# happierpig/flashinfer-ai

Hardware: AMD Instinct MI355X
Metric: paged_decode_hbm_bandwidth_bs64_kv8192_hd128 (higher is better)
Workload: dtype bf16; 1 GPU; C2: BatchDecodeWithPagedKVCacheWrapper bf16 GQA 32/8 head_dim=128 page_size=16 bs=64/GPU kv_len=8192, random page permutation; batch_per_gpu=64, kv_len=8192, num_qo_heads=32, num_kv_heads=8, head_dim=128, page_size=16, split_kv=True, kv_chunk_size=4096, parallelism=batch-shard x1 (no data-path collective)

## Files before the change

flashinfer-ai_amd/csrc/decode.hip:

```cpp
#include <stdlib.h>
#include <string.h>

#include <algorithm>
#include <vector>

#include "decode_kernel.h"
#include "merge_kernel.h"

namespace fi {

#define FI_DECL(DT, HD)                                                                   \
  hipError_t decode_launch_##DT##_##HD(const DecodeKernelParams& p, int gt, int rope, int grid, \
                                       hipStream_t stream);
FI_DECL(0, 64) FI_DECL(0, 128) FI_DECL(0, 256) FI_DECL(0, 512)
FI_DECL(1, 64) FI_DECL(1, 128) FI_DECL(1, 256) FI_DECL(1, 512)
FI_DECL(2, 64) FI_DECL(2, 128) FI_DECL(2, 256) FI_DECL(2, 512)
FI_DECL(3, 64) FI_DECL(3, 128) FI_DECL(3, 256) FI_DECL(3, 512)
#undef FI_DECL

typedef hipError_t (*decode_launch_fn)(const DecodeKernelParams&, int, int, int, hipStream_t);

static decode_launch_fn find_launcher(int kv_dt, int head_dim) {
#define FI_ROW(DT)                          \
  case DT:                                  \
    switch (head_dim) {                     \
      case 64:                              \
        return decode_launch_##DT##_64;     \
      case 128:                             \
        return decode_launch_##DT##_128;    \
      case 256:                             \
        return decode_launch_##DT##_256;    \
      case 512:                             \
        return decode_launch_##DT##_512;    \
      default:                              \
        return nullptr;                     \
    }
  switch (kv_dt) {
    FI_ROW(0)
    FI_ROW(1)
    FI_ROW(2)
    FI_ROW(3)
    default:
      return nullptr;
  }
#undef FI_ROW
}

static bool decode_mfma16() {
  static const bool on = [] {
    const char* e = getenv("FI_DECODE_MFMA16");
    return !e || atoi(e) != 0;
  }();
  return on;
}

static int decode_waves_per_cu(int kv_dtype, bool batch) {
  const bool fp8 = kv_dtype == FI_DTYPE_FP8_E4M3 || kv_dtype == FI_DTYPE_FP8_E5M2;
  return (batch && !fp8) ? 4 : 8;
}

static int tokens_per_load(int kv_dt, int head_dim) {
  const int vec = 16 / (int)dtype_size(kv_dt);
  return 64 / (head_dim / vec);
}

static int ilog2_exact(int x) {
  if (x <= 0 || (x & (x - 1))) return -1;
  int l = 0;
  while ((1 << l) < x) ++l;
  return l;
}

hipError_t decode_mfma_launch(const DecodeKernelParams& p, int q_dtype, int kv_dtype, int head_dim, int rope, int grid,
                              hipStream_t stream);
hipError_t decode_mfma16_launch(const DecodeKernelParams& p, int q_dtype, int kv_dtype, int head_dim, int rope,
                                int grid, hipStream_t stream);

constexpr int kMfmaMinGroup = 5;
constexpr int kMfmaMinGroupFp8 = 3;

enum class DecodeKernel { VALU, MFMA32, MFMA16 };

struct DecodeChoice {
  DecodeKernel kind;
  int head_tiles;
  int gt;
};

static DecodeChoice choose_decode(int group, int q_dt, int kv_dt, int head_dim, int page_size, bool rope,
                                  bool plain_logits, bool strides_fit_31_bits) {
  DecodeChoice c;
  c.gt = group <= 1 ? 1 : group == 2 ? 2 : 4;
  const bool fp8 = kv_dt == FI_DTYPE_FP8_E4M3 || kv_dt == FI_DTYPE_FP8_E5M2;
  const bool mfma = (q_dt == FI_DTYPE_F16 || q_dt == FI_DTYPE_BF16) && (kv_dt == q_dt || fp8) &&
                    (head_dim == 64 || head_dim == 128) && strides_fit_31_bits;
  if (decode_mfma16()) {
    c.kind = !(mfma && (plain_logits || group <= 16)) ? DecodeKernel::VALU
             : group <= 16                            ? DecodeKernel::MFMA16
                                                      : DecodeKernel::MFMA32;
  } else {
    const bool small_pages = ilog2_exact(page_size) < 0 || page_size < tokens_per_load(kv_dt, head_dim);
    const int min_group = (rope || small_pages) ? 1 : fp8 ? kMfmaMinGroupFp8 : kMfmaMinGroup;
    c.kind = mfma && plain_logits && group >= min_group ? DecodeKernel::MFMA32 : DecodeKernel::VALU;
  }
  c.head_tiles = c.kind == DecodeKernel::VALU ? ceil_div(group, c.gt) : ceil_div(group, 32);
  return c;
}

static int launch_decode(const DecodeKernelParams& kp, const DecodeChoice& c, int q_dt, int kv_dt, int head_dim,
                         bool rope, int merge_n, int merge_rows, hipStream_t stream) {
  if (kp.num_items > 0) {
    const int grid = ceil_div(kp.num_items, kDecodeWaves);
    if (c.kind == DecodeKernel::MFMA16)
      FI_HIP_CALL(decode_mfma16_launch(kp, q_dt, kv_dt, head_dim, rope, grid, stream));
    else if (c.kind == DecodeKernel::MFMA32)
      FI_HIP_CALL(decode_mfma_launch(kp, q_dt, kv_dt, head_dim, rope, grid, stream));
    else
      FI_HIP_CALL(find_launcher(kv_dt, head_dim)(kp, c.gt, rope, grid, stream));
  }
  if (kp.split_kv) {
    MergeNParams mp{kp.tmp_o, kp.tmp_lse, kp.o_indptr, kp.o, kp.lse, merge_n, merge_rows,
                    kp.num_qo_heads, head_dim, FI_DTYPE_F32, q_dt};
    FI_HIP_CALL(launch_merge_n(mp, stream));
  }
  return 0;
}

static int32_t window_pages(const int32_t* indptr_h, int i, int page_size, int window_left) {
  const int32_t np = indptr_h[i + 1] - indptr_h[i];
  if (window_left < 0 || np <= 0) return np;
  const int64_t first = std::max<int64_t>((int64_t)(np - 1) * page_size - window_left, 0) / page_size;
  return (int32_t)(np - first);
}

struct DecodeWork {
  bool split_kv;
  uint32_t pages_per_chunk;
  size_t padded;
};

static DecodeWork estimate_decode_work(const int32_t* indptr_h, int batch_size, int page_size, int window_left,
                                       uint32_t gdy, uint32_t max_grid, bool enable_cuda_graph) {
  std::vector<int32_t> num_pages(batch_size);
  uint32_t max_pages = 0;
  for (int i = 0; i < batch_size; ++i)
    max_pages = std::max<uint32_t>(max_pages, num_pages[i] = window_pages(indptr_h, i, page_size, window_left));
  if ((uint64_t)batch_size * gdy >= max_grid) return {false, std::max(max_pages, 1u), (size_t)batch_size};
  const uint32_t min_pages = std::max<uint32_t>(128u / (uint32_t)page_size, 1u);
  const uint32_t pages_per_chunk = (uint32_t)smallest_fitting(min_pages, max_pages, [&](int64_t pages) {
    uint64_t nb = 0;
    for (int32_t e : num_pages) nb += ceil_div<uint32_t>((uint32_t)e, (uint32_t)pages);
    return nb * gdy > max_grid;
  });
  uint32_t new_batch = 0;
  for (int32_t e : num_pages) new_batch += ceil_div<uint32_t>((uint32_t)std::max(e, 1), pages_per_chunk);
  if (enable_cuda_graph) return {true, pages_per_chunk, std::max<size_t>(max_grid / gdy, new_batch)};
  return {new_batch != (uint32_t)batch_size, pages_per_chunk, new_batch};
}

}

using namespace fi;

extern "C" FI_API int fi_batch_decode_plan(void* float_ws, size_t float_ws_bytes, void* int_ws,
                                    void* pinned_int_ws, size_t int_ws_bytes,
                                    const int32_t* indptr_h, int32_t batch_size,
                                    int32_t num_qo_heads, int32_t num_kv_heads, int32_t page_size,
                                    int32_t enable_cuda_graph, int32_t head_dim, int32_t q_dtype,
                                    int32_t kv_dtype, int32_t max_grid_hint, int32_t window_left,
                                    int64_t* plan_info_out, fi_stream_t stream) {
  (void)float_ws;
  FI_REQUIRE(pinned_int_ws && indptr_h && plan_info_out, "batch_decode_plan: null argument");
  FI_REQUIRE(batch_size >= 0 && page_size > 0, "batch_decode_plan: bad batch_size/page_size");
  FI_REQUIRE(num_kv_heads > 0 && num_qo_heads % num_kv_heads == 0,
             "batch_decode_plan: num_qo_heads (%d) must be a multiple of num_kv_heads (%d)",
             num_qo_heads, num_kv_heads);
  FI_REQUIRE(q_dtype == FI_DTYPE_F16 || q_dtype == FI_DTYPE_BF16,
             "batch_decode_plan: q dtype must be f16/bf16");
  FI_REQUIRE(find_launcher(kv_dtype, head_dim) != nullptr,
             "batch_decode_plan: unsupported kv dtype %d / head_dim %d", kv_dtype, head_dim);
  for (int i = 0; i < batch_size; ++i)
    FI_REQUIRE(indptr_h[i + 1] >= indptr_h[i], "batch_decode_plan: indptr must be non-decreasing");

  const int head_tiles = choose_decode(num_qo_heads / num_kv_heads, q_dtype, kv_dtype, head_dim, page_size,
                                       false, true, true)
                             .head_tiles;
  const uint32_t gdy = (uint32_t)(num_kv_heads * head_tiles);
  const uint32_t max_grid =
      max_grid_hint > 0 ? (uint32_t)max_grid_hint
                        : (uint32_t)(fi_num_compute_units() * decode_waves_per_cu(kv_dtype, true) * (head_tiles > 1 ? 2 : 1));

  if (window_left < 0) window_left = -1;
  const auto [split_kv, pages_per_chunk, padded] =
      estimate_decode_work(indptr_h, batch_size, page_size, window_left, gdy, max_grid, enable_cuda_graph);

  OffsetAllocator ia(int_ws_bytes);
  const int64_t req_off = ia.alloc(padded * sizeof(int32_t));
  const int64_t tile_off = ia.alloc(padded * sizeof(int32_t));
  const int64_t oind_off = ia.alloc(((size_t)batch_size + 1) * sizeof(int32_t));
  const int64_t chunk_off = ia.alloc(sizeof(int32_t));
  int64_t mask_off = 0;
  if (split_kv) mask_off = ia.alloc(padded);
  FI_REQUIRE(ia.ok, "batch_decode_plan: int workspace too small (%zu bytes)", int_ws_bytes);

  char* hp = (char*)pinned_int_ws;
  int32_t* req_h = (int32_t*)(hp + req_off);
  int32_t* tile_h = (int32_t*)(hp + tile_off);
  int32_t* oind_h = (int32_t*)(hp + oind_off);
  memset(req_h, 0, padded * sizeof(int32_t));
  memset(tile_h, 0, padded * sizeof(int32_t));
  size_t w = 0;
  oind_h[0] = 0;
  for (int b = 0; b < batch_size; ++b) {
    const uint32_t np = (uint32_t)std::max(window_pages(indptr_h, b, page_size, window_left), 1);
    const uint32_t nchunks = split_kv ? ceil_div(np, pages_per_chunk) : 1u;
    for (uint32_t t = 0; t < nchunks; ++t) {
      FI_REQUIRE(w < padded, "batch_decode_plan: work list overflow");
      req_h[w] = b;
      tile_h[w] = (int32_t)t;
      ++w;
    }
    oind_h[b + 1] = oind_h[b] + (int32_t)nchunks;
  }
  *(int32_t*)(hp + chunk_off) = (int32_t)(pages_per_chunk * (uint32_t)page_size);
  if (split_kv) {
    uint8_t* mask_h = (uint8_t*)(hp + mask_off);
    for (size_t i = 0; i < padded; ++i) mask_h[i] = i < w;
  }

  int64_t v_off = 0, s_off = 0;
  if (split_kv) {
    OffsetAllocator fa(float_ws_bytes);
    v_off = fa.alloc((size_t)num_qo_heads * padded * head_dim * sizeof(float));
    s_off = fa.alloc((size_t)num_qo_heads * padded * sizeof(float));
    FI_REQUIRE(fa.ok, "batch_decode_plan: float workspace too small (%zu bytes, need %zu)",
               float_ws_bytes, (size_t)num_qo_heads * padded * (head_dim + 1) * sizeof(float));
  }

  for (int i = 0; i < FI_DECODE_PLAN_INFO_LEN; ++i) plan_info_out[i] = 0;
  plan_info_out[FI_DP_PADDED_BATCH_SIZE] = (int64_t)padded;
  plan_info_out[FI_DP_V_OFFSET] = v_off;
  plan_info_out[FI_DP_S_OFFSET] = s_off;
  plan_info_out[FI_DP_REQUEST_INDICES_OFFSET] = req_off;
  plan_info_out[FI_DP_KV_TILE_INDICES_OFFSET] = tile_off;
  plan_info_out[FI_DP_O_INDPTR_OFFSET] = oind_off;
  plan_info_out[FI_DP_BLOCK_VALID_MASK_OFFSET] = mask_off;
  plan_info_out[FI_DP_KV_CHUNK_SIZE_PTR_OFFSET] = chunk_off;
  plan_info_out[FI_DP_ENABLE_CUDA_GRAPH] = enable_cuda_graph ? 1 : 0;
  plan_info_out[FI_DP_SPLIT_KV] = split_kv ? 1 : 0;
  plan_info_out[FI_DP_KV_CHUNK_SIZE] = (int64_t)pages_per_chunk * page_size;
  plan_info_out[FI_DP_NUM_WORK] = (int64_t)w;
  plan_info_out[FI_DP_BATCH_SIZE] = batch_size;
  plan_info_out[FI_DP_INT_BYTES_USED] = (int64_t)ia.used;
  plan_info_out[FI_DP_WINDOW_LEFT] = window_left;
  plan_info_out[FI_DP_MAGIC] = FI_DECODE_PLAN_MAGIC;

  if (int_ws && ia.used)
    FI_HIP_CALL(hipMemcpyAsync(int_ws, pinned_int_ws, ia.used, hipMemcpyHostToDevice,
                               (hipStream_t)stream));
  return 0;
}

namespace fi {

template <class A>
static int check_and_fill_decode(const char* who, const A& a, int kv_dt, int head_dim, int num_kv_heads,
                                 int page_size, int64_t kv_stride_page, int64_t kv_stride_n, int64_t kv_stride_h,
                                 DecodeKernelParams& kp, DecodeChoice& choice) {
  FI_REQUIRE(a.q_dtype == FI_DTYPE_F16 || a.q_dtype == FI_DTYPE_BF16, "%s: q dtype must be f16/bf16", who);
  FI_REQUIRE(num_kv_heads > 0 && a.num_qo_heads % num_kv_heads == 0,
             "%s: num_qo_heads must be a multiple of num_kv_heads", who);
  FI_REQUIRE(find_launcher(kv_dt, head_dim), "%s: unsupported kv dtype %d / head_dim %d", who, kv_dt, head_dim);
  FI_REQUIRE(a.pos_encoding_mode != FI_POS_ALIBI || a.alibi_slopes, "%s: ALIBI needs alibi_slopes", who);
  memset(&kp, 0, sizeof(kp));
  kp.q = a.q;
  kp.o = a.o;
  kp.lse = a.lse;
  kp.alibi_slopes = a.alibi_slopes;
  kp.kv_stride_page = kv_stride_page;
  kp.kv_stride_n = kv_stride_n;
  kp.kv_stride_h = kv_stride_h;
  kp.num_qo_heads = a.num_qo_heads;
  kp.num_kv_heads = num_kv_heads;
  kp.group_size = a.num_qo_heads / num_kv_heads;
  kp.page_size = page_size;
  kp.log2_page_size = ilog2_exact(page_size);
  kp.uniform_page = kp.log2_page_size >= 0 && page_size >= tokens_per_load(kv_dt, head_dim);
  kp.page_div = FastDiv((uint32_t)page_size);
  kp.window_left = a.window_left;
  kp.q_dtype = a.q_dtype;
  kp.use_alibi = a.pos_encoding_mode == FI_POS_ALIBI;
  kp.logits_soft_cap = a.logits_soft_cap > 0.f ? a.logits_soft_cap : 0.f;
  kp.sm_scale = a.sm_scale;
  kp.rope_rcp_scale = a.rope_rcp_scale;
  kp.rope_rcp_theta = a.rope_rcp_theta;
  const bool plain_logits = a.pos_encoding_mode != FI_POS_ALIBI && !(a.logits_soft_cap > 0.f);
  choice = choose_decode(kp.group_size, a.q_dtype, kv_dt, head_dim, page_size,
                         a.pos_encoding_mode == FI_POS_ROPE_LLAMA, plain_logits,
                         kv_stride_page < (1ll << 31) && kv_stride_n < (1ll << 31));
  kp.head_tiles = choice.head_tiles;
  return 0;
}

}

extern "C" FI_API int fi_batch_decode_run(void* float_ws, size_t float_ws_bytes, void* int_ws,
                                   size_t int_ws_bytes, const int64_t* plan_info,
                                   int32_t plan_info_len, const fi_batch_decode_params_t* a,
                                   fi_stream_t stream_) {
  hipStream_t stream = (hipStream_t)stream_;
  FI_REQUIRE(plan_info && plan_info_len == FI_DECODE_PLAN_INFO_LEN &&
                 plan_info[FI_DP_MAGIC] == FI_DECODE_PLAN_MAGIC,
             "batch_decode_run: plan_info is not a decode plan (call plan() first)");
  FI_REQUIRE(a && a->q && a->o && a->kv.k_data && a->kv.v_data && a->kv.indptr &&
                 a->kv.last_page_len,
             "batch_decode_run: null tensor");
  FI_REQUIRE(int_ws, "batch_decode_run: null int workspace");
  const fi_paged_kv_t& kv = a->kv;
  FI_REQUIRE(kv.batch_size == plan_info[FI_DP_BATCH_SIZE],
             "batch_decode_run: batch size %d differs from the planned %lld", kv.batch_size,
             (long long)plan_info[FI_DP_BATCH_SIZE]);
  FI_REQUIRE(a->pos_encoding_mode >= 0 && a->pos_encoding_mode <= 2,
             "batch_decode_run: bad pos_encoding_mode %d", a->pos_encoding_mode);
  DecodeKernelParams kp;
  DecodeChoice choice;
  if (check_and_fill_decode("batch_decode_run", *a, kv.dtype, kv.head_dim, kv.num_kv_heads, kv.page_size,
                            kv.stride_page, kv.stride_n, kv.stride_h, kp, choice))
    return 1;
  const size_t esz = dtype_size(kv.dtype);
  FI_REQUIRE(((uintptr_t)a->q % 16) == 0 && (a->q_stride_n * 2) % 16 == 0 && (a->q_stride_h * 2) % 16 == 0,
             "batch_decode_run: q rows must be 16-byte aligned");
  FI_REQUIRE((kv.stride_n * esz) % 16 == 0 && (kv.stride_h * esz) % 16 == 0 &&
                 (kv.stride_page * esz) % 16 == 0 && ((uintptr_t)kv.k_data % 16) == 0 &&
                 ((uintptr_t)kv.v_data % 16) == 0,
             "batch_decode_run: kv cache rows must be 16-byte aligned");
  if (kv.batch_size == 0) return 0;

  const bool split = plan_info[FI_DP_SPLIT_KV] != 0;
  const int64_t padded = plan_info[FI_DP_PADDED_BATCH_SIZE];
  kp.k = kv.k_data;
  kp.v = kv.v_data;
  kp.indptr = kv.indptr;
  kp.indices = kv.indices;
  kp.last_page_len = kv.last_page_len;
  const char* ib = (const char*)int_ws;
  kp.request_indices = (const int32_t*)(ib + plan_info[FI_DP_REQUEST_INDICES_OFFSET]);
  kp.kv_tile_indices = (const int32_t*)(ib + plan_info[FI_DP_KV_TILE_INDICES_OFFSET]);
  kp.o_indptr = (const int32_t*)(ib + plan_info[FI_DP_O_INDPTR_OFFSET]);
  kp.block_valid_mask =
      (split && plan_info[FI_DP_ENABLE_CUDA_GRAPH])
          ? (const uint8_t*)(ib + plan_info[FI_DP_BLOCK_VALID_MASK_OFFSET])
          : nullptr;
  (void)int_ws_bytes;
  kp.q_rope_offset = a->q_rope_offset;
  kp.kv_rope_pos_offset = kv.rope_pos_offset;
  kp.q_stride_n = a->q_stride_n;
  kp.q_stride_h = a->q_stride_h;
  kp.num_items = (int32_t)(padded * kv.num_kv_heads * kp.head_tiles);
  kp.kv_chunk_size = (int32_t)plan_info[FI_DP_KV_CHUNK_SIZE];
  kp.kv_chunk_size_ptr = (const int32_t*)(ib + plan_info[FI_DP_KV_CHUNK_SIZE_PTR_OFFSET]);
  kp.split_kv = split;
  kp.plan_window_left = (int32_t)plan_info[FI_DP_WINDOW_LEFT];
  FI_REQUIRE(kp.plan_window_left < 0 || kp.plan_window_left == a->window_left,
             "batch_decode_run: window_left %d differs from the planned %d", a->window_left, kp.plan_window_left);
  if (split) {
    FI_REQUIRE(float_ws, "batch_decode_run: split-kv plan needs the float workspace");
    const size_t need = (size_t)plan_info[FI_DP_S_OFFSET] +
                        (size_t)a->num_qo_heads * padded * sizeof(float);
    FI_REQUIRE(need <= float_ws_bytes, "batch_decode_run: float workspace too small");
    kp.tmp_o = (float*)((char*)float_ws + plan_info[FI_DP_V_OFFSET]);
    kp.tmp_lse = (float*)((char*)float_ws + plan_info[FI_DP_S_OFFSET]);
  }
  kp.fast_path = kp.uniform_page && kp.indices && !kp.use_alibi && kp.logits_soft_cap == 0.f;
  return launch_decode(kp, choice, a->q_dtype, kv.dtype, kv.head_dim, a->pos_encoding_mode == FI_POS_ROPE_LLAMA,
                       0, kv.batch_size, stream);
}

extern "C" FI_API int fi_single_decode_run(const fi_single_decode_params_t* a, void* tmp, size_t tmp_bytes,
                                    fi_stream_t stream_) {
  hipStream_t stream = (hipStream_t)stream_;
  FI_REQUIRE(a && a->q && a->k && a->v && a->o, "single_decode_run: null tensor");
  FI_REQUIRE(a->kv_len >= 0, "single_decode_run: negative kv_len");
  const int vpage = 16;
  DecodeKernelParams kp;
  DecodeChoice choice;
  if (check_and_fill_decode("single_decode_run", *a, a->kv_dtype, a->head_dim, a->num_kv_heads, vpage,
                            (int64_t)vpage * a->kv_stride_n, a->kv_stride_n, a->kv_stride_h, kp, choice))
    return 1;
  const size_t esz = dtype_size(a->kv_dtype);
  FI_REQUIRE(((uintptr_t)a->q % 16) == 0 && (a->q_stride_h * 2) % 16 == 0,
             "single_decode_run: q rows must be 16-byte aligned");
  FI_REQUIRE((a->kv_stride_n * esz) % 16 == 0 && (a->kv_stride_h * esz) % 16 == 0 &&
                 ((uintptr_t)a->k % 16) == 0 && ((uintptr_t)a->v % 16) == 0,
             "single_decode_run: k/v rows must be 16-byte aligned");

  kp.k = a->k;
  kp.v = a->v;
  kp.q_stride_n = 0;
  kp.q_stride_h = a->q_stride_h;
  kp.single_kv_len = a->kv_len;
  kp.plan_window_left = -1;
  const int gdy = a->num_kv_heads * kp.head_tiles;
  const int max_grid = fi_num_compute_units() * decode_waves_per_cu(a->kv_dtype, false);
  int chunk = a->kv_len, nchunks = 1;
  if (a->kv_len > 256 && tmp) {
    const int want = std::max(1, max_grid / gdy);
    chunk = std::max(ceil_div(a->kv_len, want), 256);
    chunk = ceil_div(chunk, vpage) * vpage;
    nchunks = ceil_div(a->kv_len, chunk);
    const size_t need = (size_t)nchunks * a->num_qo_heads * (a->head_dim + 1) * sizeof(float) + 64;
    if (need > tmp_bytes || nchunks <= 1) {
      chunk = a->kv_len;
      nchunks = 1;
    }
  }
  kp.split_kv = nchunks > 1;
  kp.kv_chunk_size = chunk;
  kp.num_items = nchunks * gdy;
  if (kp.split_kv) {
    kp.tmp_o = (float*)tmp;
    size_t vbytes = (size_t)nchunks * a->num_qo_heads * a->head_dim * sizeof(float);
    vbytes = (vbytes + 15) / 16 * 16;
    kp.tmp_lse = (float*)((char*)tmp + vbytes);
  }
  return launch_decode(kp, choice, a->q_dtype, a->kv_dtype, a->head_dim, a->pos_encoding_mode == FI_POS_ROPE_LLAMA,
                       nchunks, 1, stream);
}
```

flashinfer-ai_amd/csrc/decode_kernel.h:

```cpp
#pragma once
#include "common.h"

namespace fi {

constexpr int kDecodeThreads = 256;
constexpr int kDecodeWaves = kDecodeThreads / 64;
constexpr float kMInit = -1.0e30f;

struct DecodeKernelParams {
  const void* q;
  void* o;
  float* lse;
  float* tmp_o;
  float* tmp_lse;
  const void* k;
  const void* v;
  const int32_t* indptr;
  const int32_t* indices;
  const int32_t* last_page_len;
  const int32_t* request_indices;
  const int32_t* kv_tile_indices;
  const int32_t* o_indptr;
  const uint8_t* block_valid_mask;
  const int32_t* q_rope_offset;
  const int32_t* kv_rope_pos_offset;
  const float* alibi_slopes;
  int64_t q_stride_n, q_stride_h;
  int64_t kv_stride_page, kv_stride_n, kv_stride_h;
  int32_t num_items;
  int32_t num_qo_heads, num_kv_heads, group_size, head_tiles;
  int32_t page_size, log2_page_size;
  int32_t uniform_page;
  int32_t fast_path;
  FastDiv page_div;
  int32_t kv_chunk_size;
  const int32_t* kv_chunk_size_ptr;
  int32_t split_kv;
  int32_t single_kv_len;
  int32_t window_left;
  int32_t plan_window_left;
  int32_t q_dtype;
  int32_t use_alibi;
  float logits_soft_cap;
  float sm_scale;
  float rope_rcp_scale, rope_rcp_theta;
};

template <bool NT>
__device__ __forceinline__ u32x4 load16(const void* base, int64_t byte_off) {
  if constexpr (NT) return __builtin_nontemporal_load((const u32x4*)((const char*)base + byte_off));
  else return *(const u32x4*)((const char*)base + byte_off);
}
template <bool NT>
__device__ __forceinline__ u32x4 load16(const char* ubase, uint32_t lane_byte_off) {
  if constexpr (NT) return __builtin_nontemporal_load((const u32x4*)(ubase + lane_byte_off));
  else return *(const u32x4*)(ubase + lane_byte_off);
}

template <int KV_DT, int HEAD_DIM, int GT, bool ROPE, bool FAST, int NLOAD, bool NT = true>
struct DecodeWave {
  using T = KVTraits<KV_DT>;
  static constexpr int VEC = T::VEC;
  static constexpr int LPT = HEAD_DIM / VEC;
  static constexpr int TPL = 64 / LPT;
  static constexpr int TILE = NLOAD * TPL;
  static_assert(LPT >= 1 && LPT <= 64 && (64 % LPT) == 0, "bad head_dim");

  const DecodeKernelParams& p;
  int lane, c, r;
  int kv_head, page_begin, kv_len, chunk_start, chunk_end, win_start;
  int64_t head_off;
  uint32_t lane_voff;
  int rope_pos0;
  float q[GT][VEC];
  float o[GT][VEC];
  float m[GT], d[GT];
  float slope_l2[GT];
  float s_scale;
  float freq[ROPE ? VEC : 1];
  float rc[ROPE ? VEC : 1], rs[ROPE ? VEC : 1];
  float dc[ROPE ? VEC : 1], ds[ROPE ? VEC : 1];

  __device__ __forceinline__ DecodeWave(const DecodeKernelParams& params) : p(params) {}

  struct Buf {
    u32x4 k[NLOAD];
    u32x4 v[NLOAD];
  };

  template <bool SCALAR>
  __device__ __forceinline__ void fetch_pages(int tile_tok0, int (&pg)[NLOAD]) const {
#pragma unroll
    for (int j = 0; j < NLOAD; ++j) {
      const int tok0 = tile_tok0 + j * TPL;
      if constexpr (SCALAR) {
        const int pi = min(tok0, chunk_end - 1) >> p.log2_page_size;
        pg[j] = p.indices[page_begin + pi];
      } else {
        const int tok = min(tok0 + r, chunk_end - 1);
        const int pi = (int)fast_div((uint32_t)tok, p.page_div);
        pg[j] = p.indices ? p.indices[page_begin + pi] : pi;
      }
    }
  }

  template <bool SCALAR>
  __device__ __forceinline__ void issue_loads(int tile_tok0, const int (&pg)[NLOAD], Buf& b) const {
#pragma unroll
    for (int j = 0; j < NLOAD; ++j) {
      const int tok0 = tile_tok0 + j * TPL;
      if constexpr (SCALAR) {
        const int page = __builtin_amdgcn_readfirstlane(pg[j]);
        const int entry0 = tok0 & (p.page_size - 1);
        const int64_t sbase =
            ((int64_t)page * p.kv_stride_page + head_off + (int64_t)entry0 * p.kv_stride_n) * T::BYTES;
        b.k[j] = load16<NT>((const char*)p.k + sbase, lane_voff);
        b.v[j] = load16<NT>((const char*)p.v + sbase, lane_voff);
      } else {
        const int tok = min(tok0 + r, chunk_end - 1);
        const int pi = (int)fast_div((uint32_t)tok, p.page_div);
        const int entry = tok - pi * p.page_size;
        const int64_t off = (int64_t)pg[j] * p.kv_stride_page + head_off +
                            (int64_t)entry * p.kv_stride_n + (int64_t)(c * VEC);
        b.k[j] = load16<NT>(p.k, off * T::BYTES);
        b.v[j] = load16<NT>(p.v, off * T::BYTES);
      }
    }
  }

  static __device__ __forceinline__ void unpack_q(const u32x4 (&raw)[VEC / 8], bool is_bf16,
                                                  float (&out)[VEC]) {
#pragma unroll
    for (int v8 = 0; v8 < VEC / 8; ++v8) {
      float a[8], b[8];
      KVTraits<FI_DTYPE_BF16>::unpack(raw[v8], a);
      KVTraits<FI_DTYPE_F16>::unpack(raw[v8], b);
#pragma unroll
      for (int i = 0; i < 8; ++i) out[8 * v8 + i] = is_bf16 ? a[i] : b[i];
    }
  }

  __device__ __forceinline__ void rope_seed(int pos) {
    if constexpr (ROPE) {
#pragma unroll
      for (int i = 0; i < VEC; ++i) {
        float e = (float)pos * freq[i];
        float sn, cs;
        sincos_ool(e, &sn, &cs);
        rc[i] = cs;
        rs[i] = sn;
      }
    }
  }
  __device__ __forceinline__ void rope_advance() {
    if constexpr (ROPE) {
#pragma unroll
      for (int i = 0; i < VEC; ++i) {
        float cn = rc[i] * dc[i] - rs[i] * ds[i];
        float sn = rs[i] * dc[i] + rc[i] * ds[i];
        rc[i] = cn;
        rs[i] = sn;
      }
    }
  }

  template <bool MASKED>
  __device__ __forceinline__ void compute(int tile_tok0, const Buf& b) {
    float s[NLOAD][GT];
#pragma unroll
    for (int j = 0; j < NLOAD; ++j) {
      float kf[VEC];
      T::unpack(b.k[j], kf);
      if constexpr (ROPE) {
        float kr[VEC];
#pragma unroll
        for (int i = 0; i < VEC; ++i) {
          float partner = lane_xor<LPT / 2>(kf[i]);
          kr[i] = kf[i] * rc[i] + ((c < LPT / 2) ? -partner : partner) * rs[i];
        }
#pragma unroll
        for (int i = 0; i < VEC; ++i) kf[i] = kr[i];
        rope_advance();
      }
      const int tok = tile_tok0 + j * TPL + r;
#pragma unroll
      for (int g = 0; g < GT; ++g) {
        f32x2 acc2 = {0.f, 0.f};
#pragma unroll
        for (int i = 0; i < VEC; i += 2) {
          f32x2 qq = {q[g][i], q[g][i + 1]};
          f32x2 kk = {kf[i], kf[i + 1]};
          acc2 = __builtin_elementwise_fma(qq, kk, acc2);
        }
        float acc = group_sum<LPT>(acc2[0] + acc2[1]);
        if constexpr (!FAST) {
          if (p.use_alibi) acc += slope_l2[g] * (float)tok;
          if (p.logits_soft_cap > 0.f) acc = fast_tanh(acc) * s_scale;
        }
        if constexpr (MASKED) {
// ... 273 lines not shown
```

flashinfer-ai_amd/csrc/decode_mfma16_kernel.h:

```cpp
#pragma once
#include "decode_kernel.h"
#include "prefill_kernel.h"

namespace fi {

template <int T16>
struct Mfma16;
template <>
struct Mfma16<FI_DTYPE_F16> {
  static __device__ __forceinline__ f32x4 mfma(MfmaType<FI_DTYPE_F16>::frag a, MfmaType<FI_DTYPE_F16>::frag b, f32x4 c) {
    return __builtin_amdgcn_mfma_f32_16x16x32_f16(a, b, c, 0, 0, 0);
  }
};
template <>
struct Mfma16<FI_DTYPE_BF16> {
  static __device__ __forceinline__ f32x4 mfma(MfmaType<FI_DTYPE_BF16>::frag a, MfmaType<FI_DTYPE_BF16>::frag b, f32x4 c) {
    return __builtin_amdgcn_mfma_f32_16x16x32_bf16(a, b, c, 0, 0, 0);
  }
};

template <bool MAX>
__device__ __forceinline__ float reduce_rows(float x) {
  const uint32_t u = __builtin_bit_cast(uint32_t, x);
  const auto r = __builtin_amdgcn_permlane16_swap(u, u, false, false);
// ... 205 lines not shown
#pragma unroll
      for (int e = 0; e < 4; ++e) {
        const float cn = rc[e4 + e] * dc4[e] - rs[e4 + e] * ds4[e];
        const float sn = rs[e4 + e] * dc4[e] + rc[e4 + e] * ds4[e];
        rc[e4 + e] = cn;
        rs[e4 + e] = sn;
      }
    }
  };
  auto write_stage = [&](const Stage& st) {
#pragma unroll
    for (int ps = 0; ps < NPASS; ++ps) {
      const int row = ps * RPP + st_row;
      if constexpr (KV_FP8) {
        u32x4 k0 = fp8x8_to_16<T16, KVS>(u32x2{st.k[ps][0], st.k[ps][1]});
        u32x4 k1 = fp8x8_to_16<T16, KVS>(u32x2{st.k[ps][2], st.k[ps][3]});
        if constexpr (ROPE) {
          k0 = rope_chunk(k0, 0);
          k1 = rope_chunk(k1, 8);
          rope_advance();
        }
        *(u32x4*)(kb + k_lds_off(row, 2 * st_ch)) = k0;
        *(u32x4*)(kb + k_lds_off(row, 2 * st_ch + 1)) = k1;
        *(u32x4*)(vb + v_lds_off(row, 2 * st_ch)) = fp8x8_to_16<T16, KVS>(u32x2{st.v[ps][0], st.v[ps][1]});
        *(u32x4*)(vb + v_lds_off(row, 2 * st_ch + 1)) = fp8x8_to_16<T16, KVS>(u32x2{st.v[ps][2], st.v[ps][3]});
      } else {
        u32x4 k0 = st.k[ps];
        if constexpr (ROPE) {
          k0 = rope_chunk(k0, 0);
          rope_advance();
        }
        *(u32x4*)(kb + k_lds_off(row, st_ch)) = k0;
        *(u32x4*)(vb + v_lds_off(row, st_ch)) = st.v[ps];
      }
      if constexpr (ROPE) __builtin_amdgcn_sched_barrier(0);
    }
  };
  int k_rd[KSTEPS];
#pragma unroll
  for (int ks = 0; ks < KSTEPS; ++ks) k_rd[ks] = k_lds_off(lc, 4 * ks + lg);
  const int q4 = lc >> 2, p4 = lc & 3;
  const int v_row = 4 * lg + q4;
  int v_rd[DBLK];
#pragma unroll
  for (int db = 0; db < DBLK; ++db) v_rd[db] = v_row * ROWB + ((db ^ v_slot_key(v_row)) << 5) + p4 * 8;

  f32x4 o_acc[DBLK];
#pragma unroll
  for (int db = 0; db < DBLK; ++db) o_acc[db] = f32x4{0.f, 0.f, 0.f, 0.f};
  float m_run = -1.0e30f, l_run = 0.f;

  const int n_tok = chunk_end - chunk_start;
  if (n_tok > 0) {
    const int ntiles = (n_tok + kTile - 1) / kTile;
    int pg[NPASS], en[NPASS];
    Stage st;
    fetch_pages(chunk_start, pg, en);
    issue_loads(pg, en, st);
    fetch_pages(chunk_start + kTile, pg, en);
    for (int t = 0; t < ntiles; ++t) {
      const int tile0 = chunk_start + t * kTile;
      if constexpr (ROPE)
        if ((t & 3) == 0) rope_seed(rope_pos0 + tile0 + st_row);
      write_stage(st);
      __builtin_amdgcn_wave_barrier();
      if (t + 1 < ntiles) {
        issue_loads(pg, en, st);
        fetch_pages(tile0 + 2 * kTile, pg, en);
      }
      f32x4 s_acc[2] = {f32x4{0.f, 0.f, 0.f, 0.f}, f32x4{0.f, 0.f, 0.f, 0.f}};
#pragma unroll
      for (int ks = 0; ks < KSTEPS; ++ks) {
#pragma unroll
        for (int h = 0; h < 2; ++h) {
          const u32x4 a = *(const u32x4*)(kb + k_rd[ks] + h * 16 * ROWB);
          s_acc[h] = Mfma16<T16>::mfma(__builtin_bit_cast(frag_t, a), qf[ks], s_acc[h]);
        }
      }
      if (general) {
#pragma unroll
        for (int h = 0; h < 2; ++h)
#pragma unroll
          for (int j = 0; j < 4; ++j) {
            float t = s_acc[h][j] * p.sm_scale;
            if (p.use_alibi) t += slope * (float)(tile0 + 16 * h + 4 * lg + j);
            if (p.logits_soft_cap > 0.f) t = p.logits_soft_cap * fast_tanh(t * inv_cap);
            s_acc[h][j] = t * kLog2e;
          }
      }
      if (tile0 + kTile > chunk_end || tile0 < win_start) {
        const int lo = win_start - tile0 - 4 * lg, hi = chunk_end - tile0 - 4 * lg;
#pragma unroll
        for (int h = 0; h < 2; ++h)
#pragma unroll
          for (int j = 0; j < 4; ++j) {
            const int row = 16 * h + j;
            s_acc[h][j] = (row >= lo && row < hi) ? s_acc[h][j] : -INFINITY;
          }
      }
      float mx = fmaxf(fmaxf(fmaxf(s_acc[0][0], s_acc[0][1]), fmaxf(s_acc[0][2], s_acc[0][3])),
                       fmaxf(fmaxf(s_acc[1][0], s_acc[1][1]), fmaxf(s_acc[1][2], s_acc[1][3])));
      mx = reduce_rows<true>(mx);
      const float m_new = fmaxf(m_run, mx * c_log2);
      const float alpha = fast_exp2(m_run - m_new);
      m_run = m_new;
      float psum = 0.f;
#pragma unroll
      for (int h = 0; h < 2; ++h)
#pragma unroll
        for (int j = 0; j < 4; ++j) {
          s_acc[h][j] = fast_exp2(__builtin_fmaf(s_acc[h][j], c_log2, -m_new));
          psum += s_acc[h][j];
        }
      l_run = l_run * alpha + psum;
      if (__any(alpha != 1.0f)) {
#pragma unroll
        for (int db = 0; db < DBLK; ++db) o_acc[db] *= alpha;
      }
      u32x4 w, wl;
#pragma unroll
      for (int h = 0; h < 2; ++h)
#pragma unroll
        for (int j2 = 0; j2 < 2; ++j2) {
          const float a = s_acc[h][2 * j2], b = s_acc[h][2 * j2 + 1];
          const uint32_t pk = pack2<T16>(a, b);
          w[2 * h + j2] = pk;
          if constexpr (T16 == FI_DTYPE_BF16) {
            const float ha = __builtin_bit_cast(float, pk << 16);
            const float hb = __builtin_bit_cast(float, pk & 0xffff0000u);
            wl[2 * h + j2] = pack2<T16>(a - ha, b - hb);
          }
        }
      const frag_t pfrag = __builtin_bit_cast(frag_t, w);
#pragma unroll
      for (int db = 0; db < DBLK; ++db) {
        const char* base = vb + v_rd[db];
        const s16x4 lo = __builtin_amdgcn_ds_read_tr16_b64_v4i16((__attribute__((address_space(3))) s16x4*)(base));
        const s16x4 hi = __builtin_amdgcn_ds_read_tr16_b64_v4i16(
            (__attribute__((address_space(3))) s16x4*)(base + 16 * ROWB));
        using s16x8 = __attribute__((ext_vector_type(8))) short;
        const s16x8 a8 = {lo[0], lo[1], lo[2], lo[3], hi[0], hi[1], hi[2], hi[3]};
        o_acc[db] = Mfma16<T16>::mfma(__builtin_bit_cast(frag_t, a8), pfrag, o_acc[db]);
        if constexpr (T16 == FI_DTYPE_BF16)
          o_acc[db] = Mfma16<T16>::mfma(__builtin_bit_cast(frag_t, a8), __builtin_bit_cast(frag_t, wl), o_acc[db]);
      }
      __builtin_amdgcn_wave_barrier();
    }
  }

  l_run = reduce_rows<false>(l_run);
  const bool empty = !(l_run > 0.f);
  const float inv = empty ? 0.f : 1.0f / l_run;
  const float lse_v = empty ? FI_NEG_INF : m_run + fast_log2(l_run);
  if (lc < G) {
    const int qo_head = head0 + lc;
    const int64_t out_row = p.split_kv ? (int64_t)(p.o_indptr ? p.o_indptr[req] : 0) + kv_tile : req;
    const int64_t ob = (out_row * p.num_qo_heads + qo_head) * D;
#pragma unroll
    for (int db = 0; db < DBLK; ++db) {
      const int d0 = 16 * db + 4 * lg;
      if (p.split_kv) {
        *(f32x4*)(p.tmp_o + ob + d0) = o_acc[db] * inv;
      } else {
        const uint32_t w0 = pack2<T16>(o_acc[db][0] * inv, o_acc[db][1] * inv);
        const uint32_t w1 = pack2<T16>(o_acc[db][2] * inv, o_acc[db][3] * inv);
        *(u32x2*)((uint16_t*)p.o + ob + d0) = u32x2{w0, w1};
      }
    }
    if (lg == 0) {
      if (p.split_kv) p.tmp_lse[out_row * p.num_qo_heads + qo_head] = lse_v;
      else if (p.lse) p.lse[out_row * p.num_qo_heads + qo_head] = lse_v;
    }
  }
}

}
```

flashinfer-ai_amd/csrc/merge.hip:

```cpp
#include "merge_kernel.h"

namespace fi {

__global__ void __launch_bounds__(kMergeThreads) merge_n_kernel(const MergeNParams p) {
  __shared__ float red[kMergeWaves][kMergeMaxPerLane + 1][64];
  const int wave = __builtin_amdgcn_readfirstlane((int)(threadIdx.x >> 6));
  const int lane = threadIdx.x & 63;
  const int64_t item = blockIdx.x;
  const int row = (int)(item / p.num_heads);
  const int head = (int)(item % p.num_heads);
  int64_t first;
  int n;
  if (p.indptr) {
    first = p.indptr[row];
    n = p.indptr[row + 1] - (int)first;
  } else {
    first = (int64_t)row * p.n_fixed;
    n = p.n_fixed;
  }
  const int D = p.head_dim;
  float mx = -1.0e30f;
  for (int j0 = 0; j0 < n; j0 += 64) {
    const int j = j0 + lane;
    if (j < n) mx = fmaxf(mx, p.s[(first + j) * p.num_heads + head]);
  }
#pragma unroll
  for (int off = 32; off > 0; off >>= 1) mx = fmaxf(mx, __shfl_xor(mx, off, 64));
  float acc[kMergeMaxPerLane];
#pragma unroll
  for (int k = 0; k < kMergeMaxPerLane; ++k) acc[k] = 0.f;
  float dsum = 0.f;
  for (int j0 = 0; j0 < n; j0 += 64) {
    const int j = j0 + lane;
    const float w_lane = j < n ? fast_exp2(p.s[(first + j) * p.num_heads + head] - mx) : 0.f;
    if (wave == 0) dsum += w_lane;
    const int cnt = min(64, n - j0);
#pragma unroll 4
    for (int jj = wave; jj < cnt; jj += kMergeWaves) {
      const float w = __shfl(w_lane, jj, 64);
      const int64_t e = (first + j0 + jj) * p.num_heads + head;
#pragma unroll
      for (int k = 0; k < kMergeMaxPerLane; ++k) {
        const int i = lane + 64 * k;
        if (i < D) acc[k] += w * load_any_float(p.v, e * D + i, p.in_dtype);
      }
    }
  }
  if (n > 1) {
#pragma unroll
    for (int k = 0; k < kMergeMaxPerLane; ++k) red[wave][k][lane] = acc[k];
    __syncthreads();
    if (wave != 0) return;
#pragma unroll
    for (int k = 0; k < kMergeMaxPerLane; ++k)
      acc[k] = red[0][k][lane] + red[1][k][lane] + red[2][k][lane] + red[3][k][lane];
  } else if (wave != 0) {
    return;
  }
#pragma unroll
  for (int off = 32; off > 0; off >>= 1) dsum += __shfl_xor(dsum, off, 64);
  const int64_t ob = ((int64_t)row * p.num_heads + head) * D;
  if (n == 0 && p.skip_empty) return;
  const bool empty = !(dsum > 0.f) || mx <= FI_NEG_INF;
  const float inv = empty ? 0.f : 1.0f / dsum;
#pragma unroll
  for (int k = 0; k < kMergeMaxPerLane; ++k) {
    const int i = lane + 64 * k;
    if (i < D) store_any_float(p.v_out, ob + i, acc[k] * inv, p.out_dtype);
  }
  if (lane == 0 && p.s_out)
    p.s_out[(int64_t)row * p.num_heads + head] = empty ? FI_NEG_INF : mx + fast_log2(dsum);
}

constexpr int kMergeInFlight = 8;
template <int VEC>
__global__ void __launch_bounds__(kMergeThreads) merge_n_f32_kernel(const MergeNParams p) {
  __shared__ float red[kMergeWaves][VEC][64];
  const int wave = __builtin_amdgcn_readfirstlane((int)(threadIdx.x >> 6));
  const int lane = threadIdx.x & 63;
  const int64_t item = blockIdx.x;
  const int row = (int)(item / p.num_heads);
  const int head = (int)(item % p.num_heads);
  int64_t first;
  int n;
  if (p.indptr) {
    first = p.indptr[row];
    n = p.indptr[row + 1] - (int)first;
  } else {
    first = (int64_t)row * p.n_fixed;
    n = p.n_fixed;
  }
  if (n == 0 && p.skip_empty) return;
  constexpr int D = 64 * VEC;
  using vec_t = __attribute__((ext_vector_type(VEC))) float;
  const float* const v = (const float*)p.v;
  float mx = -1.0e30f;
  for (int j0 = 0; j0 < n; j0 += 64) {
    const int j = j0 + lane;
    if (j < n) mx = fmaxf(mx, p.s[(first + j) * p.num_heads + head]);
  }
#pragma unroll
  for (int off = 32; off > 0; off >>= 1) mx = fmaxf(mx, __shfl_xor(mx, off, 64));
  float acc[VEC];
#pragma unroll
  for (int i = 0; i < VEC; ++i) acc[i] = 0.f;
  float dsum = 0.f;
  for (int j0 = 0; j0 < n; j0 += 64) {
    const int j = j0 + lane;
    const float w_lane = j < n ? fast_exp2(p.s[(first + j) * p.num_heads + head] - mx) : 0.f;
    if (wave == 0) dsum += w_lane;
    const int cnt = min(64, n - j0);
    for (int jj0 = wave; jj0 < cnt; jj0 += kMergeWaves * kMergeInFlight) {
      float vals[kMergeInFlight][VEC], ws[kMergeInFlight];
#pragma unroll
      for (int u = 0; u < kMergeInFlight; ++u) {
        const int jj = jj0 + kMergeWaves * u;
        const int jc = min(jj, cnt - 1);
        const int64_t e = (first + j0 + jc) * p.num_heads + head;
        if constexpr (VEC == 1) {
          vals[u][0] = v[e * D + lane];
        } else {
          const vec_t t = *(const vec_t*)(v + e * D + lane * VEC);
#pragma unroll
          for (int i = 0; i < VEC; ++i) vals[u][i] = t[i];
        }
        const float w = __shfl(w_lane, jc, 64);
        ws[u] = jj < cnt ? w : 0.f;
      }
#pragma unroll
      for (int u = 0; u < kMergeInFlight; ++u)
#pragma unroll
        for (int i = 0; i < VEC; ++i) acc[i] = __builtin_fmaf(ws[u], vals[u][i], acc[i]);
    }
  }
  if (n > 1) {
#pragma unroll
    for (int i = 0; i < VEC; ++i) red[wave][i][lane] = acc[i];
    __syncthreads();
    if (wave != 0) return;
#pragma unroll
    for (int i = 0; i < VEC; ++i) acc[i] = red[0][i][lane] + red[1][i][lane] + red[2][i][lane] + red[3][i][lane];
  } else if (wave != 0) {
    return;
  }
#pragma unroll
  for (int off = 32; off > 0; off >>= 1) dsum += __shfl_xor(dsum, off, 64);
  const int64_t ob = ((int64_t)row * p.num_heads + head) * D + lane * VEC;
  const bool empty = !(dsum > 0.f) || mx <= FI_NEG_INF;
  const float inv = empty ? 0.f : 1.0f / dsum;
#pragma unroll
  for (int i = 0; i < VEC; ++i) store_any_float(p.v_out, ob + i, acc[i] * inv, p.out_dtype);
  if (lane == 0 && p.s_out)
    p.s_out[(int64_t)row * p.num_heads + head] = empty ? FI_NEG_INF : mx + fast_log2(dsum);
}

__global__ void __launch_bounds__(kMergeThreads) merge_2_kernel(const Merge2Params p) {
  const int wave = __builtin_amdgcn_readfirstlane((int)(threadIdx.x >> 6));
  const int lane = threadIdx.x & 63;
  const int64_t item = (int64_t)blockIdx.x * kMergeWaves + wave;
  if (item >= (int64_t)p.seq_len * p.num_heads) return;
  const int row = (int)(item / p.num_heads);
  if (p.mask && !p.mask[row]) return;
  const float sa = p.s_a[item], sb = p.s_b[item];
  const float mx = fmaxf(sa, sb);
  const float wa = fast_exp2(sa - mx), wb = fast_exp2(sb - mx);
  const float inv = 1.0f / (wa + wb);
  const float a_scale = wa * inv, b_scale = wb * inv;
  const int D = p.head_dim;
  const int64_t base = item * D;
  for (int i = lane; i < D; i += 64) {
    float va = load_any_float(p.v_a, base + i, p.dtype);
    float vb = load_any_float(p.v_b, base + i, p.dtype);
    store_any_float(p.v_out, base + i, a_scale * va + b_scale * vb, p.dtype);
  }
  if (lane == 0 && p.s_out) p.s_out[item] = fast_log2(wa + wb) + mx;
}


hipError_t launch_merge_n(const MergeNParams& p, hipStream_t stream) {
  const int64_t items = (int64_t)p.seq_len * p.num_heads;
  if (items == 0) return hipSuccess;
  const int grid = (int)items;
  if (p.in_dtype == FI_DTYPE_F32 && ((uintptr_t)p.v % 16) == 0) {
    switch (p.head_dim) {
      case 64: merge_n_f32_kernel<1><<<dim3(grid), dim3(kMergeThreads), 0, stream>>>(p); return hipGetLastError();
      case 128: merge_n_f32_kernel<2><<<dim3(grid), dim3(kMergeThreads), 0, stream>>>(p); return hipGetLastError();
      case 256: merge_n_f32_kernel<4><<<dim3(grid), dim3(kMergeThreads), 0, stream>>>(p); return hipGetLastError();
      default: break;
    }
  }
  merge_n_kernel<<<dim3(grid), dim3(kMergeThreads), 0, stream>>>(p);
  return hipGetLastError();
}

hipError_t launch_merge_2(const Merge2Params& p, hipStream_t stream) {
  const int64_t items = (int64_t)p.seq_len * p.num_heads;
  if (items == 0) return hipSuccess;
  const int grid = (int)((items + kMergeWaves - 1) / kMergeWaves);
  merge_2_kernel<<<dim3(grid), dim3(kMergeThreads), 0, stream>>>(p);
  return hipGetLastError();
}

static bool merge_dtype_ok(int dt) {
  return dt == FI_DTYPE_F16 || dt == FI_DTYPE_BF16 || dt == FI_DTYPE_F32;
}

}

using namespace fi;

extern "C" FI_API int fi_merge_state(const void* v_a, const float* s_a, const void* v_b, const float* s_b,
                              void* v_merged, float* s_merged, int32_t seq_len, int32_t num_heads,
                              int32_t head_dim, int32_t dtype, fi_stream_t stream) {
  if (seq_len == 0 || num_heads == 0) return 0;
  FI_REQUIRE(v_a && s_a && v_b && s_b && v_merged, "merge_state: null tensor");
  FI_REQUIRE(merge_dtype_ok(dtype), "merge_state: unsupported dtype %d", dtype);
  FI_REQUIRE(head_dim > 0 && head_dim <= 64 * kMergeMaxPerLane, "merge_state: head_dim %d unsupported", head_dim);
  Merge2Params p{v_a, s_a, v_b, s_b, v_merged, s_merged, nullptr, seq_len, num_heads, head_dim, dtype};
  FI_HIP_CALL(launch_merge_2(p, (hipStream_t)stream));
  return 0;
}

extern "C" FI_API int fi_merge_state_in_place(void* v, float* s, const void* v_other, const float* s_other,
                                       const uint8_t* mask, int32_t seq_len, int32_t num_heads,
                                       int32_t head_dim, int32_t dtype, fi_stream_t stream) {
  if (seq_len == 0 || num_heads == 0) return 0;
  FI_REQUIRE(v && s && v_other && s_other, "merge_state_in_place: null tensor");
  FI_REQUIRE(merge_dtype_ok(dtype), "merge_state_in_place: unsupported dtype %d", dtype);
  FI_REQUIRE(head_dim > 0 && head_dim <= 64 * kMergeMaxPerLane, "merge_state_in_place: head_dim %d unsupported", head_dim);
  Merge2Params p{v, s, v_other, s_other, v, s, mask, seq_len, num_heads, head_dim, dtype};
  FI_HIP_CALL(launch_merge_2(p, (hipStream_t)stream));
  return 0;
}

extern "C" FI_API int fi_merge_states(const void* v, const float* s, void* v_merged, float* s_merged,
                               int32_t num_index_sets, int32_t seq_len, int32_t num_heads,
                               int32_t head_dim, int32_t dtype, fi_stream_t stream) {
  if (seq_len == 0 || num_heads == 0) return 0;
  FI_REQUIRE((v && s || num_index_sets == 0) && v_merged, "merge_states: null tensor");
  FI_REQUIRE(merge_dtype_ok(dtype), "merge_states: unsupported dtype %d", dtype);
  FI_REQUIRE(head_dim > 0 && head_dim <= 64 * kMergeMaxPerLane, "merge_states: head_dim %d unsupported", head_dim);
  FI_REQUIRE(num_index_sets >= 0, "merge_states: negative num_index_sets");
  MergeNParams p{v, s, nullptr, v_merged, s_merged, num_index_sets, seq_len, num_heads, head_dim, dtype, dtype};
  FI_HIP_CALL(launch_merge_n(p, (hipStream_t)stream));
  return 0;
// ... 15 lines not shown
```

flashinfer-ai_amd/csrc/merge_kernel.h:

```cpp
#pragma once
#include "common.h"

namespace fi {

constexpr int kMergeThreads = 256;
constexpr int kMergeWaves = kMergeThreads / 64;
constexpr int kMergeMaxPerLane = 8;

struct MergeNParams {
  const void* v;
  const float* s;
  const int32_t* indptr;
  void* v_out;
  float* s_out;
  int32_t n_fixed;
  int32_t seq_len, num_heads, head_dim;
  int32_t in_dtype, out_dtype;
  int32_t skip_empty;
};

struct Merge2Params {
  const void* v_a;
  const float* s_a;
  const void* v_b;
  const float* s_b;
  void* v_out;
  float* s_out;
  const uint8_t* mask;
  int32_t seq_len, num_heads, head_dim, dtype;
};

hipError_t launch_merge_n(const MergeNParams& p, hipStream_t stream);
hipError_t launch_merge_2(const Merge2Params& p, hipStream_t stream);

}
```

Baseline: 6616 GB/s.

## Fuse split-KV merge into MFMA16 decode via last-arriver atomic counters

Adds per-(request, kv_head) atomic counters in the int workspace, zeroed during plan. When a request has at most four KV chunks, each MFMA16 decode block publishes its partial output and LSE, and the last block to arrive merges all partials and writes the final bf16 output directly. When the plan is known and no request exceeds the fuse limit, the separate merge kernel launch is skipped, which removes a launch and the re-read of the partial buffers. The cost is atomics and fences in the decode tail, a host-side plan cache keyed on the workspace pointer, and correctness that depends on the counters being reset by plan.

```diff
diff --git a/flashinfer-ai_amd/csrc/decode.hip b/flashinfer-ai_amd/csrc/decode.hip
--- a/flashinfer-ai_amd/csrc/decode.hip
+++ b/flashinfer-ai_amd/csrc/decode.hip
@@ -2,6 +2,8 @@
 #include <string.h>
 
 #include <algorithm>
+#include <mutex>
+#include <unordered_map>
 #include <vector>
 
 #include "decode_kernel.h"
@@ -107,8 +109,46 @@
   return c;
 }
 
+struct MergeCounterBlock {
+  size_t offset, bytes;
+  bool fits;
+};
+static MergeCounterBlock merge_counter_block(int64_t int_bytes_used, int64_t batch_size, int num_kv_heads,
+                                             size_t int_ws_bytes) {
+  MergeCounterBlock b;
+  b.offset = ((size_t)int_bytes_used + 15) / 16 * 16;
+  b.bytes = ((size_t)batch_size * num_kv_heads * sizeof(uint32_t) + 15) / 16 * 16;
+  b.fits = b.offset + b.bytes <= int_ws_bytes;
+  return b;
+}
+
+struct DecodePlanNote {
+  int64_t plan_info[FI_DECODE_PLAN_INFO_LEN];
+  int32_t max_chunks, num_kv_heads;
+};
+static std::mutex g_plan_notes_mutex;
+static std::unordered_map<const void*, DecodePlanNote> g_plan_notes;
+
+static void remember_decode_plan(const void* int_ws, const int64_t* plan_info, int max_chunks, int num_kv_heads) {
+  DecodePlanNote note;
+  memcpy(note.plan_info, plan_info, sizeof(note.plan_info));
+  note.max_chunks = max_chunks;
+  note.num_kv_heads = num_kv_heads;
+  std::lock_guard<std::mutex> lock(g_plan_notes_mutex);
+  if (g_plan_notes.size() >= 1024 && !g_plan_notes.count(int_ws)) g_plan_notes.clear();
+  g_plan_notes[int_ws] = note;
+}
+
+static bool recall_decode_plan(const void* int_ws, const int64_t* plan_info, DecodePlanNote& note) {
+  std::lock_guard<std::mutex> lock(g_plan_notes_mutex);
+  const auto it = g_plan_notes.find(int_ws);
+  if (it == g_plan_notes.end() || memcmp(it->second.plan_info, plan_info, sizeof(note.plan_info)) != 0) return false;
+  note = it->second;
+  return true;
+}
+
 static int launch_decode(const DecodeKernelParams& kp, const DecodeChoice& c, int q_dt, int kv_dt, int head_dim,
-                         bool rope, int merge_n, int merge_rows, hipStream_t stream) {
+                         bool rope, int merge_n, int merge_rows, hipStream_t stream, bool merge_launch = true) {
   if (kp.num_items > 0) {
     const int grid = ceil_div(kp.num_items, kDecodeWaves);
     if (c.kind == DecodeKernel::MFMA16)
@@ -118,9 +158,9 @@
     else
       FI_HIP_CALL(find_launcher(kv_dt, head_dim)(kp, c.gt, rope, grid, stream));
   }
-  if (kp.split_kv) {
+  if (kp.split_kv && merge_launch) {
     MergeNParams mp{kp.tmp_o, kp.tmp_lse, kp.o_indptr, kp.o, kp.lse, merge_n, merge_rows,
-                    kp.num_qo_heads, head_dim, FI_DTYPE_F32, q_dt};
+                    kp.num_qo_heads, head_dim, FI_DTYPE_F32, q_dt, 0, kp.fuse_max};
     FI_HIP_CALL(launch_merge_n(mp, stream));
   }
   return 0;
@@ -210,6 +250,7 @@
   memset(req_h, 0, padded * sizeof(int32_t));
   memset(tile_h, 0, padded * sizeof(int32_t));
   size_t w = 0;
+  uint32_t max_chunks = 0;
   oind_h[0] = 0;
   for (int b = 0; b < batch_size; ++b) {
     const uint32_t np = (uint32_t)std::max(window_pages(indptr_h, b, page_size, window_left), 1);
@@ -221,6 +262,7 @@
       ++w;
     }
     oind_h[b + 1] = oind_h[b] + (int32_t)nchunks;
+    max_chunks = std::max(max_chunks, nchunks);
   }
   *(int32_t*)(hp + chunk_off) = (int32_t)(pages_per_chunk * (uint32_t)page_size);
   if (split_kv) {
@@ -255,9 +297,13 @@
   plan_info_out[FI_DP_WINDOW_LEFT] = window_left;
   plan_info_out[FI_DP_MAGIC] = FI_DECODE_PLAN_MAGIC;
 
-  if (int_ws && ia.used)
+  if (int_ws && ia.used) {
     FI_HIP_CALL(hipMemcpyAsync(int_ws, pinned_int_ws, ia.used, hipMemcpyHostToDevice,
                                (hipStream_t)stream));
+    const MergeCounterBlock cb = merge_counter_block((int64_t)ia.used, batch_size, num_kv_heads, int_ws_bytes);
+    if (cb.fits && cb.bytes) FI_HIP_CALL(hipMemsetAsync((char*)int_ws + cb.offset, 0, cb.bytes, (hipStream_t)stream));
+    remember_decode_plan(int_ws, plan_info_out, (int)max_chunks, num_kv_heads);
+  }
   return 0;
 }
 
@@ -351,7 +397,6 @@
       (split && plan_info[FI_DP_ENABLE_CUDA_GRAPH])
           ? (const uint8_t*)(ib + plan_info[FI_DP_BLOCK_VALID_MASK_OFFSET])
           : nullptr;
-  (void)int_ws_bytes;
   kp.q_rope_offset = a->q_rope_offset;
   kp.kv_rope_pos_offset = kv.rope_pos_offset;
   kp.q_stride_n = a->q_stride_n;
@@ -372,8 +417,20 @@
     kp.tmp_lse = (float*)((char*)float_ws + plan_info[FI_DP_S_OFFSET]);
   }
   kp.fast_path = kp.uniform_page && kp.indices && !kp.use_alibi && kp.logits_soft_cap == 0.f;
+  bool merge_launch = true;
+  if (split && choice.kind == DecodeKernel::MFMA16) {
+    const MergeCounterBlock cb =
+        merge_counter_block(plan_info[FI_DP_INT_BYTES_USED], kv.batch_size, kv.num_kv_heads, int_ws_bytes);
+    DecodePlanNote note;
+    const bool known = recall_decode_plan(int_ws, plan_info, note);
+    if (cb.fits && !(known && note.num_kv_heads != kv.num_kv_heads)) {
+      kp.merge_counters = (uint32_t*)((char*)int_ws + cb.offset);
+      kp.fuse_max = kDecodeFuseMax;
+      merge_launch = plan_info[FI_DP_ENABLE_CUDA_GRAPH] != 0 || !known || note.max_chunks > kDecodeFuseMax;
+    }
+  }
   return launch_decode(kp, choice, a->q_dtype, kv.dtype, kv.head_dim, a->pos_encoding_mode == FI_POS_ROPE_LLAMA,
-                       0, kv.batch_size, stream);
+                       0, kv.batch_size, stream, merge_launch);
 }
 
 extern "C" FI_API int fi_single_decode_run(const fi_single_decode_params_t* a, void* tmp, size_t tmp_bytes,
diff --git a/flashinfer-ai_amd/csrc/decode_kernel.h b/flashinfer-ai_amd/csrc/decode_kernel.h
--- a/flashinfer-ai_amd/csrc/decode_kernel.h
+++ b/flashinfer-ai_amd/csrc/decode_kernel.h
@@ -6,6 +6,7 @@
 constexpr int kDecodeThreads = 256;
 constexpr int kDecodeWaves = kDecodeThreads / 64;
 constexpr float kMInit = -1.0e30f;
+constexpr int kDecodeFuseMax = 4;
 
 struct DecodeKernelParams {
   const void* q;
@@ -44,7 +45,18 @@
   float logits_soft_cap;
   float sm_scale;
   float rope_rcp_scale, rope_rcp_theta;
+  uint32_t* merge_counters;
+  int32_t fuse_max;
 };
+
+template <int COUNT>
+__device__ __forceinline__ float merge_weight_tree(const float* w, int base, int stride) {
+  static_assert(COUNT >= 1 && COUNT <= 64 && (COUNT & (COUNT - 1)) == 0, "a power of two");
+  if constexpr (COUNT == 1)
+    return w[base];
+  else
+    return merge_weight_tree<COUNT / 2>(w, base, 2 * stride) + merge_weight_tree<COUNT / 2>(w, base + stride, 2 * stride);
+}
 
 template <bool NT>
 __device__ __forceinline__ u32x4 load16(const void* base, int64_t byte_off) {
diff --git a/flashinfer-ai_amd/csrc/decode_mfma16_kernel.h b/flashinfer-ai_amd/csrc/decode_mfma16_kernel.h
--- a/flashinfer-ai_amd/csrc/decode_mfma16_kernel.h
+++ b/flashinfer-ai_amd/csrc/decode_mfma16_kernel.h
@@ -381,25 +381,101 @@
   const bool empty = !(l_run > 0.f);
   const float inv = empty ? 0.f : 1.0f / l_run;
   const float lse_v = empty ? FI_NEG_INF : m_run + fast_log2(l_run);
+  const int64_t first_row = p.split_kv && p.o_indptr ? p.o_indptr[req] : 0;
+  int n_fused = 0;
+  if (p.split_kv && p.fuse_max > 0) {
+    const int n = p.o_indptr[req + 1] - (int)first_row;
+    if (n <= p.fuse_max) n_fused = n;
+  }
+  const bool final_out = !p.split_kv || n_fused == 1;
+  const bool publish = n_fused >= 2;
+  const uint32_t entry_bytes = (uint32_t)p.num_qo_heads * D * 4u;
+  const auto part_rsrc = __builtin_amdgcn_make_buffer_rsrc(
+      (void*)(p.tmp_o + (publish ? (first_row * p.num_qo_heads + head0) * D : 0)), 0,
+      publish ? (int)((uint32_t)(n_fused - 1) * entry_bytes + (uint32_t)G * D * 4u) : 0, 0x00020000);
+  constexpr int kWriteThrough = 16;
   if (lc < G) {
     const int qo_head = head0 + lc;
-    const int64_t out_row = p.split_kv ? (int64_t)(p.o_indptr ? p.o_indptr[req] : 0) + kv_tile : req;
+    const int64_t out_row = final_out ? req : first_row + kv_tile;
     const int64_t ob = (out_row * p.num_qo_heads + qo_head) * D;
 #pragma unroll
     for (int db = 0; db < DBLK; ++db) {
       const int d0 = 16 * db + 4 * lg;
-      if (p.split_kv) {
+      if (final_out) {
+        f32x4 x = o_acc[db] * inv;
+        if (p.split_kv) x = x + 0.0f;
+        const uint32_t w0 = pack2<T16>(x[0], x[1]);
+        const uint32_t w1 = pack2<T16>(x[2], x[3]);
+        *(u32x2*)((uint16_t*)p.o + ob + d0) = u32x2{w0, w1};
+      } else if (publish) {
+        __builtin_amdgcn_raw_buffer_store_b128(
+            __builtin_bit_cast(u32x4, o_acc[db] * inv), part_rsrc,
+            (uint32_t)kv_tile * entry_bytes + (uint32_t)((lc * D + d0) * 4), 0, kWriteThrough);
+      } else {
         *(f32x4*)(p.tmp_o + ob + d0) = o_acc[db] * inv;
+      }
+    }
+    if (lg == 0) {
+      if (final_out) {
+        if (p.lse) p.lse[out_row * p.num_qo_heads + qo_head] = lse_v;
+      } else if (publish) {
+        __hip_atomic_store(p.tmp_lse + out_row * p.num_qo_heads + qo_head, lse_v, __ATOMIC_RELAXED,
+                           __HIP_MEMORY_SCOPE_AGENT);
       } else {
-        const uint32_t w0 = pack2<T16>(o_acc[db][0] * inv, o_acc[db][1] * inv);
-        const uint32_t w1 = pack2<T16>(o_acc[db][2] * inv, o_acc[db][3] * inv);
-        *(u32x2*)((uint16_t*)p.o + ob + d0) = u32x2{w0, w1};
-      }
-    }
-    if (lg == 0) {
-      if (p.split_kv) p.tmp_lse[out_row * p.num_qo_heads + qo_head] = lse_v;
-      else if (p.lse) p.lse[out_row * p.num_qo_heads + qo_head] = lse_v;
-    }
+        p.tmp_lse[out_row * p.num_qo_heads + qo_head] = lse_v;
+      }
+    }
+  }
+  if (!publish) return;
+
+  asm volatile("s_waitcnt vmcnt(0)" ::: "memory");
+  uint32_t drawn = 0;
+  if (lane == 0)
+    drawn = atomicInc(p.merge_counters + (int64_t)req * p.num_kv_heads + kv_head, (uint32_t)(n_fused - 1));
+  const int ticket = __builtin_amdgcn_readfirstlane((int)drawn);
+  if (ticket != n_fused - 1) return;
+  __builtin_amdgcn_fence(__ATOMIC_ACQUIRE, "agent");
+  asm volatile("s_waitcnt vmcnt(0)" ::: "memory");
+  if (lc < G) {
+    const int qo_head = head0 + lc;
+    float w[kDecodeFuseMax];
+#pragma unroll
+    for (int j = 0; j < kDecodeFuseMax; ++j)
+      w[j] = __hip_atomic_load(p.tmp_lse + (first_row + min(j, n_fused - 1)) * p.num_qo_heads + qo_head,
+                               __ATOMIC_RELAXED, __HIP_MEMORY_SCOPE_AGENT);
+    f32x4 part[kDecodeFuseMax][DBLK];
+#pragma unroll
+    for (int j = 0; j < kDecodeFuseMax; ++j) {
+      const uint32_t off = j < n_fused ? (uint32_t)j * entry_bytes + (uint32_t)((lc * D + 4 * lg) * 4) : 0x80000000u;
+#pragma unroll
+      for (int db = 0; db < DBLK; ++db)
+        part[j][db] = __builtin_bit_cast(
+            f32x4, __builtin_amdgcn_raw_buffer_load_b128(part_rsrc, off + 64 * db, 0, kWriteThrough));
+    }
+    float mx = -1.0e30f;
+#pragma unroll
+    for (int j = 0; j < kDecodeFuseMax; ++j) mx = fmaxf(mx, w[j]);
+#pragma unroll
+    for (int j = 0; j < kDecodeFuseMax; ++j) w[j] = j < n_fused ? fast_exp2(w[j] - mx) : 0.f;
+    const float dsum = merge_weight_tree<kDecodeFuseMax>(w, 0, 1);
+    const bool none = !(dsum > 0.f) || mx <= FI_NEG_INF;
+    const float inv_d = none ? 0.f : 1.0f / dsum;
+    const int64_t ob = ((int64_t)req * p.num_qo_heads + qo_head) * D;
+#pragma unroll
+    for (int db = 0; db < DBLK; ++db) {
+      f32x4 chain[4];
+#pragma unroll
+      for (int c = 0; c < 4; ++c) chain[c] = f32x4{0.f, 0.f, 0.f, 0.f};
+#pragma unroll
+      for (int j = 0; j < kDecodeFuseMax; ++j)
+#pragma unroll
+        for (int e = 0; e < 4; ++e) chain[j & 3][e] = __builtin_fmaf(w[j], part[j][db][e], chain[j & 3][e]);
+      const f32x4 x = (((chain[0] + chain[1]) + chain[2]) + chain[3]) * inv_d;
+      const uint32_t w0 = pack2<T16>(x[0], x[1]);
+      const uint32_t w1 = pack2<T16>(x[2], x[3]);
+      *(u32x2*)((uint16_t*)p.o + ob + 16 * db + 4 * lg) = u32x2{w0, w1};
+    }
+    if (lg == 0 && p.lse) p.lse[(int64_t)req * p.num_qo_heads + qo_head] = none ? FI_NEG_INF : mx + fast_log2(dsum);
   }
 }
 
diff --git a/flashinfer-ai_amd/csrc/merge.hip b/flashinfer-ai_amd/csrc/merge.hip
--- a/flashinfer-ai_amd/csrc/merge.hip
+++ b/flashinfer-ai_amd/csrc/merge.hip
@@ -18,6 +18,7 @@
     first = (int64_t)row * p.n_fixed;
     n = p.n_fixed;
   }
+  if (n > 0 && n <= p.skip_upto) return;
   const int D = p.head_dim;
   float mx = -1.0e30f;
   for (int j0 = 0; j0 < n; j0 += 64) {
@@ -91,6 +92,7 @@
     n = p.n_fixed;
   }
   if (n == 0 && p.skip_empty) return;
+  if (n > 0 && n <= p.skip_upto) return;
   constexpr int D = 64 * VEC;
   using vec_t = __attribute__((ext_vector_type(VEC))) float;
   const float* const v = (const float*)p.v;
diff --git a/flashinfer-ai_amd/csrc/merge_kernel.h b/flashinfer-ai_amd/csrc/merge_kernel.h
--- a/flashinfer-ai_amd/csrc/merge_kernel.h
+++ b/flashinfer-ai_amd/csrc/merge_kernel.h
@@ -17,6 +17,7 @@
   int32_t seq_len, num_heads, head_dim;
   int32_t in_dtype, out_dtype;
   int32_t skip_empty;
+  int32_t skip_upto;
 };
 
 struct Merge2Params {
```

Result: no change. 6626 GB/s (median of 6 runs) (+0.2%).
